# tohtsky/myFM

Hardware: AMD Instinct MI355X
Metric: Gibbs iterations/sec (rank=32) (higher is better)
Workload: dtype f64

## Files before the change

include/myfm_hip.h:

```cpp
#ifndef MYFM_HIP_H_
#define MYFM_HIP_H_

#include <stdint.h>

#ifdef __cplusplus
extern "C" {
#endif

#define MFM_OK 0
#define MFM_ERR_INVALID 1
#define MFM_ERR_RUNTIME 2
#define MFM_ERR_DEVICE 3

#define MFM_TASK_REGRESSION 0
#define MFM_TASK_CLASSIFICATION 1
#define MFM_TASK_ORDERED 2

typedef struct mfm_ctx mfm_ctx;
typedef struct mfm_design mfm_design;
typedef struct mfm_store mfm_store;

const char *mfm_version(void);
int mfm_device_count(void);
const char *mfm_global_error(void);
// ... 13 lines not shown
int mfm_comm_info(const mfm_ctx *ctx, int32_t *n_ranks, char *path, int64_t path_cap);
int mfm_peer_info(mfm_ctx *ctx, int32_t *pending, void **sum_buf, void **flag_buf, int64_t *sum_bytes, int64_t *flag_bytes);
int mfm_peer_set(mfm_ctx *ctx, int32_t world, int32_t rank, void *const *sum_bufs, void *const *flag_bufs);
int mfm_peer_model_info(mfm_ctx *ctx, void **w_buf, void **V_buf);
int mfm_peer_set_model(mfm_ctx *ctx, int32_t world, int32_t rank, void *const *w_bufs, void *const *V_bufs);
int mfm_peer_export(mfm_ctx *ctx, void *handles256);
int mfm_peer_import(mfm_ctx *ctx, int32_t world, int32_t rank, const void *all_handles);
int mfm_peer_drop(mfm_ctx *ctx);
int mfm_set_main_levels(mfm_ctx *ctx, const int32_t *level, int64_t D0);
int mfm_set_row_offset(mfm_ctx *ctx, int64_t first_global_row);

int mfm_set_main(mfm_ctx *ctx, int64_t N, int64_t D0, const int64_t *indptr, const int32_t *indices,
                 const double *data, const double *y);
int mfm_add_block(mfm_ctx *ctx, int64_t B, int64_t Db, const int64_t *indptr, const int32_t *indices,
                  const double *data, const int64_t *original_to_block);
int mfm_set_groups(mfm_ctx *ctx, const int32_t *group_index, int64_t D, int32_t G);
int mfm_set_residual_policy(mfm_ctx *ctx, int32_t recomputable);
int mfm_finalize(mfm_ctx *ctx, int32_t rank);

int64_t mfm_dim_all(const mfm_ctx *ctx);
int mfm_plan_info(const mfm_ctx *ctx, int64_t *n_levels_main, int64_t *n_launches_per_sweep);
int mfm_plan_flags(const mfm_ctx *ctx);
#define MFM_RES_INFO_FIELDS 16
int mfm_res_info(const mfm_ctx *ctx, int64_t *out, int n_out, char *why, int why_len);
#define MFM_CELL_INFO_FIELDS 74
int mfm_cell_info(const mfm_ctx *ctx, int64_t *out, int n_out, char *why, int why_len);
#define MFM_CHAIN_STREAM_INFO_FIELDS 30
int mfm_chain_stream_info(const mfm_ctx *ctx, int64_t *out, int max_records, int *n_records);

int mfm_set_state(mfm_ctx *ctx, double w0, const double *w, const double *V);
int mfm_get_state(mfm_ctx *ctx, double *w0, double *w, double *V);
int mfm_set_w0(mfm_ctx *ctx, double w0);
int mfm_zero_w(mfm_ctx *ctx);
int mfm_get_e(mfm_ctx *ctx, double *e);
int mfm_get_q(mfm_ctx *ctx, double *q);
int mfm_set_e(mfm_ctx *ctx, const double *e);

int mfm_reduce_e(mfm_ctx *ctx, double *sum_e, double *sum_e2);
int mfm_shift_e(mfm_ctx *ctx, double delta);
int mfm_group_stats_w(mfm_ctx *ctx, const double *mu_w, double *sum, double *ssd);
int mfm_group_stats_V(mfm_ctx *ctx, const double *mu_V, double *sum, double *ssd);
int mfm_hyper_stats(mfm_ctx *ctx, int32_t need_e, const double *mu_w, const double *mu_V, double *sum_e, double *sum_e2,
                    double *sum_w, double *ssd_w, double *sum_V, double *ssd_V);
int mfm_sweep_w(mfm_ctx *ctx, double alpha, const double *lambda_w, const double *mu_w, const double *z);
int mfm_sweep_V(mfm_ctx *ctx, int32_t f_begin, int32_t f_end, double alpha, const double *lambda_V,
                const double *mu_V, const double *z);
// ... 280 lines not shown
```

myfm_amd/_build.py:

```python
import os
import subprocess
import sys
import sysconfig

HERE = os.path.dirname(os.path.abspath(__file__))
ROOT = os.path.dirname(HERE)
CSRC = os.path.join(HERE, "csrc")
INCLUDE = os.path.join(ROOT, "include")
HIP_LIB = os.path.join(HERE, "libmyfm_hip.so")
EXT_SUFFIX = sysconfig.get_config_var("EXT_SUFFIX") or ".so"
PYMOD = os.path.join(HERE, "_myfm" + EXT_SUFFIX)

HIP_UNITS = {
    "mfm_hip.hip": ["mfm_env.hpp", "mfm_common.hpp", "mfm_wave.hpp", "mfm_policies.hpp", "mfm_kernels.hpp", "mfm_mf_kernels.hpp", "mfm_res.hpp", "mfm_res_entry.hpp", "mfm_res_plan.hpp",
                    "mfm_plan.hpp", "mfm_block_kernels.hpp", "mfm_erfcx.hpp", "mfm_tasks.hpp", "mfm_tn.hpp", "mfm_philox.hpp", "mfm_predict.hpp", "mfm_samples.hpp", "mfm_dist.hpp", "mfm_logdens.hpp", "mfm_psis.hpp", "mfm_ess.hpp", "mfm_crps.hpp", "mfm_loo_pred.hpp", "mfm_normal_quantile.hpp", "mfm_rng.hpp", "mfm_mtjump.hpp", "mfm_cell.hpp",
                    "mfm_chain_api.hpp", "mfm_rng_state.hpp", "mfm_latent_api.hpp", "mfm_latent_host.hpp", "mfm_comm.hpp", "mfm_vbmoments.hpp", "mfm_vb_sums.hpp"],
    "mfm_latent.hip": ["mfm_env.hpp", "mfm_common.hpp", "mfm_rng_state.hpp", "mfm_latent_api.hpp"],
    "mfm_cell.hip": ["mfm_env.hpp", "mfm_common.hpp", "mfm_wave.hpp", "mfm_cell.hpp"],
    "mfm_chain.hip": ["mfm_env.hpp", "mfm_common.hpp", "mfm_wave.hpp", "mfm_policies.hpp", "mfm_chain_api.hpp", "mfm_chain_plan.hpp", "mfm_chain_stream.hpp"],
    "mfm_vb.hip": ["mfm_env.hpp", "mfm_common.hpp", "mfm_erfcx.hpp", "mfm_vb.hpp", "mfm_comm.hpp"],
    "mfm_pairs.hip": ["mfm_env.hpp", "mfm_common.hpp", "mfm_pairs.hpp", "mfm_pairs_rank.hpp", "mfm_pairs_samples.hpp", "mfm_pairs_ucb.hpp", "mfm_pairs_vb.hpp", "mfm_vb_sums.hpp", "mfm_samples.hpp"],
    "mfm_foldin.hip": ["mfm_env.hpp", "mfm_common.hpp", "mfm_foldin.hpp", "mfm_foldin_handle.hpp", "mfm_philox.hpp", "mfm_samples.hpp"],
    "mfm_foldin_gibbs.hip": ["mfm_env.hpp", "mfm_common.hpp", "mfm_foldin.hpp", "mfm_foldin_gibbs.hpp", "mfm_foldin_gibbs_plan.hpp",
                             "mfm_foldin_handle.hpp", "mfm_tn.hpp", "mfm_philox.hpp", "mfm_samples.hpp"],
}
OBJ_DIR = os.path.join(CSRC, "_obj")
PYMOD_HEADERS = ["mfm_env.hpp", "mfm_hostnormals.hpp", "mfm_mtjump.hpp", "mfm_normal_quantile.hpp"]


def _newer(target, deps):
    if not os.path.exists(target):
        return True
    t = os.path.getmtime(target)
    return any(os.path.exists(d) and os.path.getmtime(d) > t for d in deps)


def _hipcc():
# ... 75 lines not shown
```

myfm_amd/_capi.py:

```python
import ctypes as C
import os

import numpy as np
import scipy.sparse as sps

_HERE = os.path.dirname(os.path.abspath(__file__))
LIB_PATH = os.path.join(_HERE, "libmyfm_hip.so")

MFM_OK, MFM_ERR_INVALID, MFM_ERR_RUNTIME, MFM_ERR_DEVICE = 0, 1, 2, 3
TASK_REGRESSION, TASK_CLASSIFICATION, TASK_ORDERED = 0, 1, 2

SYMBOLS = [
    "mfm_version", "mfm_device_count", "mfm_global_error", "mfm_create", "mfm_destroy", "mfm_last_error",
    "mfm_set_stream", "mfm_synchronize", "mfm_set_main", "mfm_add_block", "mfm_set_groups", "mfm_finalize",
    "mfm_peer_info", "mfm_peer_set", "mfm_peer_model_info", "mfm_peer_set_model", "mfm_peer_export", "mfm_peer_import", "mfm_peer_drop", "mfm_set_residual_policy", "mfm_dim_all", "mfm_plan_info", "mfm_plan_flags", "mfm_res_info", "mfm_cell_info", "mfm_chain_stream_info", "mfm_set_state", "mfm_get_state", "mfm_set_w0", "mfm_zero_w", "mfm_get_e",
    "mfm_get_q", "mfm_set_e", "mfm_reduce_e", "mfm_shift_e", "mfm_group_stats_w", "mfm_group_stats_V",
    "mfm_sweep_w", "mfm_sweep_V", "mfm_sweep_wV", "mfm_update_e_regression", "mfm_update_e_classification", "mfm_score_train",
    "mfm_oprobit_add_group", "mfm_oprobit_eval", "mfm_oprobit_sample_z", "mfm_hyper_stats", "mfm_timing_enable", "mfm_timing_select", "mfm_timing_reset",
    "mfm_timing_n_classes", "mfm_timing_class_name", "mfm_timing_get", "mfm_design_create", "mfm_design_add_block",
    "mfm_design_destroy", "mfm_design_last_error", "mfm_design_dim_all", "mfm_design_predict",
    "mfm_host_column_levels", "mfm_rng_prepare", "mfm_rng_seed_mt19937", "mfm_rng_set_program", "mfm_rng_prefetch", "mfm_rng_acquire",
    "mfm_rng_get_z", "mfm_design_score_ctx", "mfm_design_n_rows", "mfm_set_allreduce", "mfm_set_row_offset", "mfm_set_main_levels",
    "mfm_test_erfcx", "mfm_test_truncated_normal", "mfm_get_device", "mfm_set_shard", "mfm_comm_unique_id", "mfm_comm_init",
    "mfm_comm_stats", "mfm_comm_info", "mfm_store_create", "mfm_store_destroy", "mfm_store_last_error", "mfm_store_size", "mfm_store_push_ctx",
# ... 475 lines not shown
    def latent_stats(self):
        out = np.zeros(8, dtype=np.int64)
        self._ck(lib().mfm_latent_stats(self.h, _p(out)))
        return dict(zip(("status", "chunks", "subs", "lq", "quads", "walkers", "attempts"), (int(v) for v in out)))

    def rng_host_read(self, offset, n):
        out = np.empty(max(int(n), 1), dtype=np.uint32)
        self._ck(lib().mfm_rng_host_read(self.h, int(offset), int(n), _p(out)))
        return out[: int(n)]

    def rng_host_advance(self, words):
        self._ck(lib().mfm_rng_host_advance(self.h, int(words)))

    def set_residual_policy(self, recomputable):
        self._ck(lib().mfm_set_residual_policy(self.h, 1 if recomputable else 0))

    def plan_flags(self):
        f = lib().mfm_plan_flags(self.h)
        return {"qfree": bool(f & 1), "unit": bool(f & 2), "ell": bool(f & 4), "sharded": bool(f & 8), "soa": bool(f & 16),
                "fused_next": bool(f & 32), "sharded_fused": bool(f & 64), "mf": bool(f & 128), "resident": bool(f & 256), "cell": bool(f & 512), "streamed_chain": bool(f & 1024), "resident_overflow": bool(f & 2048)}

    RES_INFO = ("ready", "G", "RV", "RL", "RX", "umax", "n_items", "item_bits", "n_runs", "max_wg_users", "max_slice_items",
                "e_where", "n_rows", "s2_in_sweep_b", "lds_bytes", "entry_bytes")
    E_WHERE = ("rows", "slots", "slots_with_sums", "cell", "dropped")

    def res_info(self):
        out = np.zeros(len(self.RES_INFO), dtype=np.int64)
        why = C.create_string_buffer(256)
        self._ck(lib().mfm_res_info(self.h, _p(out), out.shape[0], why, len(why)))
        d = dict(zip(self.RES_INFO, (int(v) for v in out)))
        d["ready"] = bool(d["ready"])
        d["e_where"] = self.E_WHERE[d["e_where"]]
        d["why"] = why.value.decode()
        return d

    CELL_INFO = ("ready", "G", "umax", "item32", "n_streams", "n_fields", "N", "Npad", "max_steps", "chunk_max", "chunk_min",
                 "chunks_empty", "split_mask", "score_fb")
    CELL_STREAM_TYPE = ("U", "I", "C")
    CELL_MAX_STREAMS, CELL_MAX_FIELDS = 4, 16
    CELL_INFO_FIELDS = len(CELL_INFO) + 3 * CELL_MAX_STREAMS + 3 * CELL_MAX_FIELDS

    def cell_info(self):
        out = np.zeros(self.CELL_INFO_FIELDS, dtype=np.int64)
        why = C.create_string_buffer(256)
        self._ck(lib().mfm_cell_info(self.h, _p(out), out.shape[0], why, len(why)))
        n = len(self.CELL_INFO)
        nf = n + 3 * self.CELL_MAX_STREAMS
        d = dict(zip(self.CELL_INFO, (int(v) for v in out[:n])))
        d["ready"], d["item32"] = bool(d["ready"]), bool(d["item32"])
        d["streams"] = [(self.CELL_STREAM_TYPE[int(out[n + 3 * s])], int(out[n + 3 * s + 1]), int(out[n + 3 * s + 2]))
                        for s in range(d["n_streams"])]
        d["fields"] = [tuple(int(x) for x in out[nf + 3 * k:nf + 3 * k + 3]) for k in range(d["n_fields"])]
        d["why"] = why.value.decode()
# ... 614 lines not shown
```

myfm_amd/csrc/_myfm.cpp:

```cpp
#include <thread>
#include <cstdio>
#include <pybind11/functional.h>
#include <pybind11/numpy.h>
#include <pybind11/pybind11.h>
#include <pybind11/stl.h>

#include <algorithm>
#include <cmath>
#include <chrono>
#include <cstdint>
#include <cstdlib>
#include <functional>
#include <limits>
#include <memory>
#include <random>
#include <set>
#include <sstream>
#include <stdexcept>
#include <string>
#include <tuple>
#include <type_traits>
#include <vector>

#include "mfm_env.hpp"
// ... 3333 lines not shown
             mfm_comm_stats(s.trainer->ctx, &c, &d);
             return py::make_tuple(c, d);
           })
      .def("comm_info",
           [](GibbsSession &s) {
             int32_t n = 0;
             char path[512];
             if (mfm_comm_info(s.trainer->ctx, &n, path, sizeof(path)) != MFM_OK) throw std::runtime_error(mfm_global_error());
             return py::make_tuple((int)n, std::string(path));
           },
           "(ranks of the library's own RCCL communicator (ncclCommCount), path of the librccl.so it bound); (0, '') without one")
      .def("step", &GibbsSession::step, py::call_guard<py::gil_scoped_release>())
      .def("synchronize", &GibbsSession::synchronize)
      .def("residual", &GibbsSession::residual)
      .def("timing_enable", &GibbsSession::timing_enable)
      .def("timing_select", &GibbsSession::timing_select)
      .def("timing_reset", &GibbsSession::timing_reset)
      .def("timing", &GibbsSession::timing)
      .def("plan_info", &GibbsSession::plan_info)
      .def("latent_info", &GibbsSession::latent_info)
      .def("plan_flags", [](GibbsSession &s) { return mfm_plan_flags(s.trainer->ctx); })
      .def("res_info",
           [](GibbsSession &s) {
             std::vector<int64_t> v(MFM_RES_INFO_FIELDS, 0);
             ck(s.trainer->ctx, mfm_res_info(s.trainer->ctx, v.data(), (int)v.size(), nullptr, 0));
             return v;
           },
           "the persistent sweep's layout: the MFM_RES_INFO_FIELDS values of mfm_res_info (myfm_hip.h)")
      .def("peer_info",
           [](GibbsSession &s) {
             int32_t pending = 0;
             void *sum = nullptr, *flag = nullptr;
             int64_t sb = 0, fb = 0;
             ck(s.trainer->ctx, mfm_peer_info(s.trainer->ctx, &pending, &sum, &flag, &sb, &fb));
             return py::make_tuple(pending != 0, (uintptr_t)sum, (uintptr_t)flag, sb, fb);
           })
      .def("peer_set",
           [](GibbsSession &s, int world, int rank, const std::vector<uintptr_t> &sums, const std::vector<uintptr_t> &flags) {
             if ((int)sums.size() != world || (int)flags.size() != world) throw std::invalid_argument("peer_set: one buffer pair per rank");
             std::vector<void *> a, b;
             for (auto v : sums) a.push_back((void *)v);
             for (auto v : flags) b.push_back((void *)v);
             ck(s.trainer->ctx, mfm_peer_set(s.trainer->ctx, world, rank, a.data(), b.data()));
           })
      .def("peer_model_info",
           [](GibbsSession &s) {
             void *w = nullptr, *V = nullptr;
             ck(s.trainer->ctx, mfm_peer_model_info(s.trainer->ctx, &w, &V));
             return py::make_tuple((uintptr_t)w, (uintptr_t)V);
           })
      .def("peer_set_model",
// ... 135 lines not shown
```

myfm_amd/csrc/mfm_hip.hip:

```cpp
#include <algorithm>
#include <cerrno>
#include <chrono>
#include <cmath>
#include <cstdio>
#include <cstring>
#include <map>
#include <memory>
#include <mutex>
#include <string>
#include <thread>
#include <type_traits>
#include <vector>

#include <fcntl.h>
#include <sys/file.h>
#include <sys/stat.h>
#include <unistd.h>

#include <hipcub/hipcub.hpp>

#include "mfm_common.hpp"
#include "mfm_kernels.hpp"
#include "mfm_plan.hpp"
#include "mfm_res_plan.hpp"
// ... 1528 lines not shown
  bool streamed = false;
  for (auto &B : ctx->blocks)
    for (const Step &st : B->plan_V.steps) streamed = streamed || (st.is_chain && st.chain.form == ChainForm::Stream);
  int form = 0;
  switch (ctx->v_path) {
    case VPath::QFree: form = 1; break;
    case VPath::Split: form = 16; break;
    case VPath::SplitFused: form = 16 | 32; break;
    case VPath::TwoField: form = 16 | 32 | 128; break;
    case VPath::ShardedSplit: form = 64; break;
    case VPath::ShardedTwoField: form = 64 | 128; break;
    case VPath::Deferred:
    case VPath::Generic:
    case VPath::Cell:
      break;
  }
  return (streamed ? 1024 : 0) | (ctx->resident_V() && ctx->res.RX > 0 ? 2048 : 0) | form | (ctx->X.unit ? 2 : 0) | (ctx->X.ell_width >= 0 ? 4 : 0) |
         (ctx->comm.active() ? 8 : 0) | (ctx->resident_V() ? 256 : 0) | (ctx->cell.ready ? 512 : 0);
}

int mfm_res_info(const mfm_ctx *ctx, int64_t *out, int n_out, char *why, int why_len) {
  if (!ctx || n_out < 0 || (n_out > 0 && !out) || why_len < 0 || (why_len > 0 && !why)) return MFM_ERR_INVALID;
  const ResPlan &rp = ctx->res;
  const int64_t v[MFM_RES_INFO_FIELDS] = {ctx->resident_V() ? 1 : 0, rp.G,       rp.RV,     rp.RL,           rp.RX,
                                          rp.umax,          rp.n_items, rp.item_bits, rp.n_runs,    rp.max_wg_users,
                                          rp.max_slice_items, (int64_t)ctx->e_where, rp.n_rows, rp.s2b, (int64_t)rp.lds_bytes,
                                          rp.ent_bytes};
  for (int i = 0; i < n_out; i++) out[i] = i < MFM_RES_INFO_FIELDS ? v[i] : 0;
  if (why_len > 0) {
    std::strncpy(why, ctx->resident_V() ? "" : rp.why.c_str(), (size_t)why_len - 1);
    why[why_len - 1] = 0;
  }
  return MFM_OK;
}

int mfm_cell_info(const mfm_ctx *ctx, int64_t *out, int n_out, char *why, int why_len) {
  if (!ctx || n_out < 0 || (n_out > 0 && !out) || why_len < 0 || (why_len > 0 && !why)) return MFM_ERR_INVALID;
  const CellPlan &cp = ctx->cell;
  int64_t v[MFM_CELL_INFO_FIELDS] = {0};
  const int m = (int)cp.fields.size(), ns = (int)cp.streams.size();
  int64_t split = 0;
  const bool typed = ns > 0 && cp.sU == 0;
  for (int k = 0; k < m && typed; k++)
    if (cp.split_pass(k == 0 ? m - 1 : k - 1, k, k == 0)) split |= (int64_t)1 << k;
  const int64_t head[14] = {cp.ready ? 1 : 0, cp.G,         cp.umax,      cp.item32 ? 1 : 0, ns,    m, cp.N, cp.Npad, cp.max_steps,
                            cp.chunk_max,     cp.chunk_min, cp.chunks_empty, split,          cp.ready ? cp.score_fb() : 0};
  for (int i = 0; i < 14; i++) v[i] = head[i];
  for (int i = 0; i < ns && i < CELL_MAX_STREAMS; i++) {
    v[14 + 3 * i] = cp.streams[i].type;
    v[15 + 3 * i] = cp.streams[i].slot;
    v[16 + 3 * i] = cp.streams[i].card;
// ... 938 lines not shown
```

myfm_amd/csrc/mfm_res.hpp:

```cpp
#pragma once
#include <algorithm>
#include <cstdlib>
#include <cstring>
#include <atomic>
#include <string>
#include <thread>
#include <type_traits>
#include <vector>

#include "mfm_common.hpp"
#include "mfm_mf_kernels.hpp"
#include "mfm_res_entry.hpp"

namespace mfm {

#ifndef MFM_RES_CH
#define MFM_RES_CH 4
#endif
constexpr int RES_MAX_PEERS = 8;

struct ResArgs {
  double2 *eq;
  const double *e_in;
  double *e_slots;
  const int32_t *perm;
  const uint32_t *uidw;
  const uint32_t *headw;
  const int32_t *run_item;
  const int32_t *first_run;
  const int32_t *wg_run_ptr;
  const int32_t *wg_nruns;
  const int32_t *wg_user_ptr;
  const int2 *user_desc;
  const int32_t *wg_item_ptr;
// ... 1045 lines not shown
  void alloc_exchange(int world, int rank, hipStream_t s) {
    xworld = world;
    xrank = rank;
    peers_set = false;
    peers_model = false;
    xepoch = 0;
    auto alloc_shared = [&](auto &buf, size_t count) {
      buf.release();
      void *p = nullptr;
      const size_t bytes = count * sizeof(*buf.p);
      if (hipExtMallocWithFlags(&p, bytes, hipDeviceMallocUncached) != hipSuccess) {
        (void)hipGetLastError();
        throw Error(MFM_ERR_DEVICE, "no uncached device memory for the ranks' exchange buffers (hipExtMallocWithFlags(hipDeviceMallocUncached))");
      }
      buf.p = (decltype(buf.p))p;
      buf.n = count;
      buf.owned = true;
      MFM_HIP_CHECK(hipMemsetAsync(p, 0, bytes, s));
    };
    alloc_shared(xsum, xsum_bytes(world) / sizeof(double));
    alloc_shared(xflag, (size_t)16 * RES_MAX_PEERS);
    xarrive.alloc_zero(16, s);
  }
  std::string why;
  std::vector<int32_t> h_nruns;
  std::vector<std::string> h_diag;

  static int bits_for(int64_t n) {
    int b = 1;
    while (((int64_t)1 << b) < n) b++;
    return b;
  }
  struct Variant {
    int rv, rl;
  };
  static std::vector<Variant> variants() {
    std::vector<Variant> v;
    for (const ResForm &f : res_forms())
      if (!f.xch && !f.ovf && !f.s2b) v.push_back({f.rv, f.rl});
    return v;
  }

  bool choose_layout(int64_t N, const std::vector<int64_t> &ustart, int64_t max_user, int n_cu, std::vector<int64_t> &ucut) {
    const int64_t n_users = (int64_t)ustart.size() - 1;
    const std::vector<Variant> vs = variants();
    const int nv = (int)vs.size();
// ... 213 lines not shown
      for (int32_t c : wg_run_item[g]) h_slot_ptr[(size_t)c + 1]++;
    }
    for (int c = 0; c < n_items; c++) h_slot_ptr[(size_t)c + 1] += h_slot_ptr[c];
    h_slot_ptr[n_items] = (int32_t)counter;
    n_runs = counter;
    if (counter >= ((int64_t)1 << 31) - 2) return fail("too many runs");
    std::vector<int32_t> run_base = run_bases(nruns);
    const int32_t zero_run = run_base[G];
    std::vector<int32_t> h_run_item((size_t)zero_run + 1, n_items);
    for (int g = 0; g < G; g++) {
      std::copy(wg_run_item[g].begin(), wg_run_item[g].end(), h_run_item.begin() + run_base[g]);
      if (fill[g] < cap_slots) {
        const int th = (int)(fill[g] / R), rh = (int)(fill[g] % R);
        h_headw[((size_t)g * HW + rh / 16) * NT + th] |= 1u << (rh % 16);
      }
      h_headw[((size_t)g * HW) * NT] |= 1u;
      for (int t = 0; t < NT; t++) {
        const int64_t s0 = (int64_t)t * R;
        int32_t &fr = h_first[(size_t)g * NT + t];
        fr = (s0 >= fill[g] ? nruns[g] : fr) + run_base[g];
      }
    }
    std::vector<int32_t> h_uptr((size_t)G + 1, 0);
    std::vector<int2> h_udesc;
    for (int g = 0; g < G; g++) {
      for (int32_t j : wg_users[g]) h_udesc.push_back(make_int2(j, group_of && (size_t)j < group_of->size() ? (*group_of)[j] : 0));
      h_uptr[g + 1] = (int32_t)h_udesc.size();
    }
    std::vector<int32_t> h_iptr;
    if (!choose_item_slices(h_slot_ptr, counter, h_iptr)) return false;
    int imax = 0;
    for (int g = 0; g < G; g++) imax = std::max(imax, h_iptr[g + 1] - h_iptr[g]);
    max_slice_items = imax;
    umax = std::max(maxu, imax) + 1;
    if (umax > 1024) return fail("internal: user field");
    std::vector<uint32_t> h_uidw((size_t)G * UW * NT, 0);
    res_parallel_for(G, [&](int g) {
      for (int64_t sl = 0; sl < cap_slots; sl++) {
        const uint16_t u16 = h_uid[(size_t)g * cap_slots + (size_t)sl];
        const uint32_t u = u16 == 0xffffu ? (uint32_t)(umax - 1) : u16;
        const int t = (int)(sl / R), r = (int)(sl % R);
        const int w0 = 5 * (r / 16), bb = (r % 16) / 4, k = r % 4;
        if (k < 3) {
          h_uidw[((size_t)g * UW + w0 + bb) * NT + t] |= u << (10 * k);
        } else {
          h_uidw[((size_t)g * UW + w0 + bb) * NT + t] |= (u & 3u) << 30;
          h_uidw[((size_t)g * UW + w0 + 4) * NT + t] |= (u >> 2) << (8 * bb);
        }
      }
    });
    h_uid = std::vector<uint16_t>();
    std::vector<int32_t> slice_of((size_t)n_items);
    for (int g = 0; g < G; g++)
      for (int c = h_iptr[g]; c < h_iptr[g + 1]; c++) slice_of[c] = g;
    std::vector<int32_t> h_eptr((size_t)G + 1, 0);
    {
      std::vector<int64_t> cnt((size_t)G, 0);
      for (int g = 0; g < G; g++)
        for (int32_t c : wg_run_item[g]) cnt[slice_of[c]]++;
      for (int g = 0; g < G; g++) {
        const int64_t e = h_eptr[g] + ((cnt[g] + WAVE - 1) / WAVE) * WAVE;
        if (e >= ((int64_t)1 << 31)) return fail("too many entries");
        h_eptr[g + 1] = (int32_t)e;
// ... 376 lines not shown
```

myfm_amd/csrc/mfm_res_plan.hpp:

```cpp
#pragma once
#include <chrono>

#include <hipcub/hipcub.hpp>

#include "mfm_res.hpp"

namespace mfm {

namespace rp {

constexpr int TB = 256;

__global__ void k_rows(const int32_t *__restrict__ colidx, int64_t N, int32_t *__restrict__ bflag, int32_t *__restrict__ ucnt,
                       int32_t *__restrict__ icnt, int32_t *__restrict__ red) {
  const int64_t r = (int64_t)blockIdx.x * blockDim.x + threadIdx.x;
  int32_t mu = -1, mi = 0x7fffffff;
  if (r < N) {
    const int2 c = ((const int2 *)colidx)[r];
    const bool b = r == 0 || c.x != colidx[2 * (r - 1)];
    bflag[r] = b ? 1 : 0;
    if (b) atomicAdd(&ucnt[c.x], 1);
    atomicAdd(&icnt[c.y], 1);
    mu = c.x;
    mi = c.y;
// ... 111 lines not shown
                       const int32_t *__restrict__ hrun0, const int32_t *__restrict__ run_base, int item_bits, int64_t N,
                       int32_t *__restrict__ run_item_c, int32_t *__restrict__ run_item, int32_t *__restrict__ runs_per_item) {
  const int64_t p = (int64_t)blockIdx.x * blockDim.x + threadIdx.x;
  if (p >= N || !headf[p]) return;
  const uint32_t k = key[p];
  const int g = (int)(k >> item_bits);
  const int32_t item = (int32_t)(k & ((1u << item_bits) - 1u));
  const int32_t kc = hs[p] - 1;
  run_item_c[kc] = item;
  run_item[run_base[g] + kc - hrun0[g]] = item;
  atomicAdd(&runs_per_item[item], 1);
}

__global__ void k_first(const int32_t *__restrict__ hs, const int32_t *__restrict__ rowcut, const int32_t *__restrict__ hrun0,
                        const int32_t *__restrict__ run_base, int G, int R, int NT, int32_t *__restrict__ first_run) {
  const int i = blockIdx.x * blockDim.x + threadIdx.x;
  if (i >= G * NT) return;
  const int g = i / NT, t = i % NT;
  const int32_t fill = rowcut[g + 1] - rowcut[g], s0 = t * R;
  const int32_t nr = hrun0[g + 1] - hrun0[g];
  first_run[i] = run_base[g] + (s0 >= fill ? nr : hs[rowcut[g] + s0] - 1 - hrun0[g]);
}

__global__ void k_pack(const uint16_t *__restrict__ uid, const int32_t *__restrict__ headf, const int32_t *__restrict__ rowcut, int G, int R,
                       int NT, int umax, uint32_t *__restrict__ uidw, uint32_t *__restrict__ headw) {
  const int HW = R / 16, UW = 5 * HW;
  const int64_t i = (int64_t)blockIdx.x * blockDim.x + threadIdx.x;
  if (i >= (int64_t)G * HW * NT) return;
  const int t = (int)(i % NT), grp = (int)((i / NT) % HW), g = (int)(i / ((int64_t)NT * HW));
  const int64_t cap = (int64_t)R * NT;
  const int32_t fill = rowcut[g + 1] - rowcut[g];
  uint32_t w[5] = {0, 0, 0, 0, 0}, hw = 0;
  for (int q = 0; q < 16; q++) {
    const int32_t sidx = t * R + 16 * grp + q;
    const uint16_t u16 = uid[(int64_t)g * cap + sidx];
    const uint32_t u = u16 == 0xffffu ? (uint32_t)(umax - 1) : u16;
    const int bb = q / 4, k = q % 4;
    if (k < 3) {
      w[bb] |= u << (10 * k);
    } else {
      w[bb] |= (u & 3u) << 30;
      w[4] |= (u >> 2) << (8 * bb);
    }
    const bool head = sidx < fill ? headf[rowcut[g] + sidx] != 0 : sidx == fill;
    if (head || sidx == 0) hw |= 1u << q;
  }
  for (int k = 0; k < 5; k++) uidw[((int64_t)g * UW + 5 * grp + k) * NT + t] = w[k];
  headw[((int64_t)g * HW + grp) * NT + t] = hw;
}

__global__ void k_user_desc(const int32_t *__restrict__ users, const int32_t *__restrict__ empties, const int32_t *__restrict__ ucut,
                            const int32_t *__restrict__ uptr, const int32_t *__restrict__ group, int G, int32_t n_users, int32_t n_emp,
                            int2 *__restrict__ desc) {
  __shared__ int32_t cut[1026];
  for (int i = threadIdx.x; i <= G; i += blockDim.x) cut[i] = ucut[i];
  __syncthreads();
  const int32_t i = blockIdx.x * blockDim.x + threadIdx.x;
  if (i < n_users) {
    const int g = upper_group(cut, G, i);
    const int32_t j = users[i];
    desc[uptr[g] + (i - cut[g])] = make_int2(j, group ? group[j] : 0);
  } else if (i < n_users + n_emp) {
    const int32_t k = i - n_users;
    const int g = k % G;
    const int32_t j = empties[k];
    desc[uptr[g] + (cut[g + 1] - cut[g]) + k / G] = make_int2(j, group ? group[j] : 0);
  }
}

__global__ void k_item_desc(const int32_t *__restrict__ scols, const int32_t *__restrict__ group, int32_t n_items, int2 *__restrict__ desc) {
  const int32_t i = blockIdx.x * blockDim.x + threadIdx.x;
  if (i < n_items) desc[i] = make_int2(scols[i], group ? group[scols[i]] : 0);
}

__global__ void k_run_feat(const int32_t *__restrict__ run_item, const int32_t *__restrict__ scols, int32_t n_items, int64_t n_run_item,
                           int64_t n, int32_t *__restrict__ run_feat) {
  const int64_t r = (int64_t)blockIdx.x * blockDim.x + threadIdx.x;
  if (r >= n) return;
  int32_t f = -1;
  if (r < n_run_item) {
    const int32_t c = run_item[r];
    if (c < n_items) f = scols[c];
  }
  run_feat[r] = f;
}

__global__ void k_slice_keys(const int32_t *__restrict__ run_item_c, const int32_t *__restrict__ iptr, int G, int64_t n, uint32_t *__restrict__ key,
                             int32_t *__restrict__ val) {
  __shared__ int32_t cut[1026];
// ... 193 lines not shown
  rpn.wg_run_ptr.upload(run_base);
  rpn.wg_nruns.upload(nruns);
  rpn.run_item.alloc((size_t)zero_run + 1);
  hipLaunchKernelGGL(k_fill32, grid(zero_run + 1), dim3(TB), 0, s, rpn.run_item.p, (int64_t)zero_run + 1, n_items);
  DevBuf<int32_t> run_item_c, runs_per_item;
  run_item_c.alloc((size_t)std::max<int64_t>(counter, 1));
  runs_per_item.alloc_zero((size_t)n_items, s);
  hipLaunchKernelGGL(k_runs, grid(N), dim3(TB), 0, s, key2.p, headf.p, hs.p, hrun0.p, rpn.wg_run_ptr.p, rpn.item_bits, N, run_item_c.p,
                     rpn.run_item.p, runs_per_item.p);
  rpn.first_run.alloc((size_t)G * NT);
  hipLaunchKernelGGL(k_first, grid((int64_t)G * NT), dim3(TB), 0, s, hs.p, rowcut.p, hrun0.p, rpn.wg_run_ptr.p, G, R, NT, rpn.first_run.p);
  lap("slots, heads, runs, first");
  std::vector<int32_t> h_slot_ptr((size_t)n_items + 1, 0), h_iptr;
  {
    const std::vector<int32_t> rpi = download(runs_per_item.p, (size_t)n_items, s);
    for (int c = 0; c < n_items; c++) h_slot_ptr[(size_t)c + 1] = h_slot_ptr[c] + rpi[c];
  }
  if (!rpn.choose_item_slices(h_slot_ptr, counter, h_iptr)) return false;
  int imax = 0;
  for (int g = 0; g < G; g++) imax = std::max(imax, h_iptr[g + 1] - h_iptr[g]);
  rpn.max_slice_items = imax;
  rpn.umax = std::max(maxu, imax) + 1;
  if (rpn.umax > 1024) return rpn.fail("internal: user field");
  const int UW = 5 * (R / 16), HW = R / 16;
  rpn.uidw.alloc((size_t)G * UW * NT);
  rpn.headw.alloc((size_t)G * HW * NT);
  hipLaunchKernelGGL(k_pack, grid((int64_t)G * HW * NT), dim3(TB), 0, s, uid.p, headf.p, rowcut.p, G, R, NT, rpn.umax, rpn.uidw.p, rpn.headw.p);
  std::vector<int32_t> h_eptr((size_t)G + 1, 0), h_sstart((size_t)G + 1, 0);
  for (int g = 0; g < G; g++) {
    const int64_t cnt = h_slot_ptr[h_iptr[g + 1]] - h_slot_ptr[h_iptr[g]];
    const int64_t e = h_eptr[g] + ((cnt + WAVE - 1) / WAVE) * WAVE;
    if (e >= ((int64_t)1 << 31)) return rpn.fail("too many entries");
    h_eptr[g + 1] = (int32_t)e;
    h_sstart[g + 1] = h_sstart[g] + (int32_t)cnt;
  }
  rpn.wg_item_ptr.upload(h_iptr);
  rpn.ent_ptr.upload(h_eptr);
  rpn.choose_entry_width(zero_run);
  const bool ent4 = rpn.ent_bytes == 4;
  rpn.entries.alloc((size_t)(rpn.ent_bytes / 4) * (size_t)h_eptr[G]);
  if (h_eptr[G]) hipLaunchKernelGGL(k_fill_entries, grid(h_eptr[G]), dim3(TB), 0, s, rpn.entries.p, (int64_t)h_eptr[G], zero_run, 0, ent4);
  if (counter > 0) {
    DevBuf<int32_t> sstart;
    sstart.upload(h_sstart);
    DevBuf<uint32_t> sk, sk2;
    DevBuf<int32_t> sv, sv2;
    sk.alloc((size_t)counter);
    sk2.alloc((size_t)counter);
    sv.alloc((size_t)counter);
    sv2.alloc((size_t)counter);
    hipLaunchKernelGGL(k_slice_keys, grid(counter), dim3(TB), 0, s, run_item_c.p, rpn.wg_item_ptr.p, G, counter, sk.p, sv.p);
    sort_pairs(sk, sk2, sv, sv2, counter, gbits, tmp, s);
    hipLaunchKernelGGL(k_entries, grid(counter), dim3(TB), 0, s, sk2.p, sv2.p, run_item_c.p, hrun0.p, rpn.wg_run_ptr.p, rpn.wg_item_ptr.p,
                       rpn.ent_ptr.p, sstart.p, G, counter, rpn.entries.p, ent4);
    MFM_HIP_CHECK(hipStreamSynchronize(s));
  }
  lap("slices, pack, entries");
  DevBuf<int32_t> d_group;
  if (group_of && (int64_t)group_of->size() >= D0) d_group.upload(group_of->data(), (size_t)D0);
  rpn.user_desc.alloc((size_t)h_uptr[G]);
  hipLaunchKernelGGL(k_user_desc, grid((int64_t)n_users + n_emp), dim3(TB), 0, s, d_users.p, empties.p, d_ucut.p, rpn.wg_user_ptr.p, d_group.p, G,
                     n_users, n_emp, rpn.user_desc.p);
  rpn.item_desc.alloc((size_t)n_items);
  hipLaunchKernelGGL(k_item_desc, grid(n_items), dim3(TB), 0, s, rpn.scols.p, d_group.p, n_items, rpn.item_desc.p);
  rpn.run_feat.alloc((size_t)zero_run + 1 + 8);
  hipLaunchKernelGGL(k_run_feat, grid((int64_t)zero_run + 9), dim3(TB), 0, s, rpn.run_item.p, rpn.scols.p, n_items, (int64_t)zero_run + 1,
                     (int64_t)zero_run + 9, rpn.run_feat.p);
  {
    std::vector<int32_t> h_fill((size_t)G);
    for (int g = 0; g < G; g++) h_fill[g] = h_rowcut[g + 1] - h_rowcut[g];
    rpn.wg_fill.upload(h_fill);
  }
  if (!rpn.plan_lds()) return rpn.fail("LDS");
  rpn.fill_s2_lin(s);
  rpn.e_slots.alloc((size_t)G * cap_slots);
  rpn.sums.alloc((size_t)G);
  rpn.y_slots = DevBuf<double>();
  rpn.h_nruns = nruns;
  rpn.h_diag.clear();
  rpn.partials.alloc((size_t)2 * ((size_t)zero_run + 1));
  MFM_HIP_CHECK(hipMemsetAsync(rpn.partials.p, 0, (size_t)16 * ((size_t)zero_run + 1), s));
  rpn.dv.alloc((size_t)rpn.dv_doubles() * (n_items + 1));
  rpn.bar.alloc(RES_BAR_WORDS);
  MFM_HIP_CHECK(hipStreamSynchronize(s));
  MFM_HIP_CHECK(hipGetLastError());
  lap("descriptors, buffers");
  rpn.ready = true;
  rpn.why.clear();
  return true;
}

static inline std::string res_plan_compare(const ResPlan &a, const ResPlan &b, hipStream_t s) {
  if (a.G != b.G || a.RV != b.RV || a.RL != b.RL || a.RX != b.RX || a.umax != b.umax || a.item_bits != b.item_bits || a.n_items != b.n_items ||
      a.n_rows != b.n_rows || a.n_runs != b.n_runs || a.lds_bytes != b.lds_bytes || a.s2b != b.s2b || a.max_wg_users != b.max_wg_users ||
      a.max_slice_items != b.max_slice_items || a.ent_bytes != b.ent_bytes)
    return "scalars";
  auto same = [&](const void *p, size_t np, const void *q, size_t nq, size_t elem) {
    if (np != nq) return false;
    std::vector<char> x(np * elem), y(nq * elem);
    if (np) {
      MFM_HIP_CHECK(hipMemcpyAsync(x.data(), p, np * elem, hipMemcpyDeviceToHost, s));
      MFM_HIP_CHECK(hipMemcpyAsync(y.data(), q, nq * elem, hipMemcpyDeviceToHost, s));
    }
    MFM_HIP_CHECK(hipStreamSynchronize(s));
    return x == y;
  };
#define MFM_RP_CMP(f) \
  if (!same(a.f.p, a.f.n, b.f.p, b.f.n, sizeof(*a.f.p))) return #f;
  MFM_RP_CMP(perm)
  MFM_RP_CMP(first_run)
  MFM_RP_CMP(wg_run_ptr)
  MFM_RP_CMP(wg_nruns)
  MFM_RP_CMP(wg_user_ptr)
  MFM_RP_CMP(wg_item_ptr)
  MFM_RP_CMP(ent_ptr)
  MFM_RP_CMP(scols)
  MFM_RP_CMP(entries)
  MFM_RP_CMP(uidw)
// ... 13 lines not shown
```

Baseline: 380.6.

## Renumber per-workgroup user slots to reduce LDS bank conflicts in resident sweep

Adds a host-side greedy assignment that renumbers each workgroup's users so their LDS positions spread across banks. It uses a model of the gfx950 LDS access groups for 64-bit reads, 128-bit reads and 64-bit atomic adds. The packed uid words and user descriptors are rewritten through this numbering, so the persistent sweep kernel's LDS accumulations conflict less. This adds planning time on the host and a device-to-host download of uid, and exposes conflict counts in res_info. An env flag can keep the identity numbering.

Result: faster. 385.1 (median of 5 runs) (+1.2%).

```diff
diff --git a/include/myfm_hip.h b/include/myfm_hip.h
--- a/include/myfm_hip.h
+++ b/include/myfm_hip.h
@@ -59,6 +59,7 @@
 int mfm_plan_info(const mfm_ctx *ctx, int64_t *n_levels_main, int64_t *n_launches_per_sweep);
 int mfm_plan_flags(const mfm_ctx *ctx);
 #define MFM_RES_INFO_FIELDS 16
+#define MFM_RES_INFO_BANK_FIELDS 2
 int mfm_res_info(const mfm_ctx *ctx, int64_t *out, int n_out, char *why, int why_len);
 #define MFM_CELL_INFO_FIELDS 74
 int mfm_cell_info(const mfm_ctx *ctx, int64_t *out, int n_out, char *why, int why_len);
diff --git a/myfm_amd/_build.py b/myfm_amd/_build.py
--- a/myfm_amd/_build.py
+++ b/myfm_amd/_build.py
@@ -12,7 +12,7 @@
 PYMOD = os.path.join(HERE, "_myfm" + EXT_SUFFIX)
 
 HIP_UNITS = {
-    "mfm_hip.hip": ["mfm_env.hpp", "mfm_common.hpp", "mfm_wave.hpp", "mfm_policies.hpp", "mfm_kernels.hpp", "mfm_mf_kernels.hpp", "mfm_res.hpp", "mfm_res_entry.hpp", "mfm_res_plan.hpp",
+    "mfm_hip.hip": ["mfm_env.hpp", "mfm_common.hpp", "mfm_wave.hpp", "mfm_policies.hpp", "mfm_kernels.hpp", "mfm_mf_kernels.hpp", "mfm_res.hpp", "mfm_res_banks.hpp", "mfm_res_entry.hpp", "mfm_res_plan.hpp",
                     "mfm_plan.hpp", "mfm_block_kernels.hpp", "mfm_erfcx.hpp", "mfm_tasks.hpp", "mfm_tn.hpp", "mfm_philox.hpp", "mfm_predict.hpp", "mfm_samples.hpp", "mfm_dist.hpp", "mfm_logdens.hpp", "mfm_psis.hpp", "mfm_ess.hpp", "mfm_crps.hpp", "mfm_loo_pred.hpp", "mfm_normal_quantile.hpp", "mfm_rng.hpp", "mfm_mtjump.hpp", "mfm_cell.hpp",
                     "mfm_chain_api.hpp", "mfm_rng_state.hpp", "mfm_latent_api.hpp", "mfm_latent_host.hpp", "mfm_comm.hpp", "mfm_vbmoments.hpp", "mfm_vb_sums.hpp"],
     "mfm_latent.hip": ["mfm_env.hpp", "mfm_common.hpp", "mfm_rng_state.hpp", "mfm_latent_api.hpp"],
diff --git a/myfm_amd/_capi.py b/myfm_amd/_capi.py
--- a/myfm_amd/_capi.py
+++ b/myfm_amd/_capi.py
@@ -521,13 +521,14 @@
 
     RES_INFO = ("ready", "G", "RV", "RL", "RX", "umax", "n_items", "item_bits", "n_runs", "max_wg_users", "max_slice_items",
                 "e_where", "n_rows", "s2_in_sweep_b", "lds_bytes", "entry_bytes")
+    RES_INFO_BANKS = ("bank_cycles_identity", "bank_cycles_chosen")
     E_WHERE = ("rows", "slots", "slots_with_sums", "cell", "dropped")
 
     def res_info(self):
-        out = np.zeros(len(self.RES_INFO), dtype=np.int64)
+        out = np.zeros(len(self.RES_INFO) + len(self.RES_INFO_BANKS), dtype=np.int64)
         why = C.create_string_buffer(256)
         self._ck(lib().mfm_res_info(self.h, _p(out), out.shape[0], why, len(why)))
-        d = dict(zip(self.RES_INFO, (int(v) for v in out)))
+        d = dict(zip(self.RES_INFO + self.RES_INFO_BANKS, (int(v) for v in out)))
         d["ready"] = bool(d["ready"])
         d["e_where"] = self.E_WHERE[d["e_where"]]
         d["why"] = why.value.decode()
diff --git a/myfm_amd/csrc/_myfm.cpp b/myfm_amd/csrc/_myfm.cpp
--- a/myfm_amd/csrc/_myfm.cpp
+++ b/myfm_amd/csrc/_myfm.cpp
@@ -3379,11 +3379,11 @@
       .def("plan_flags", [](GibbsSession &s) { return mfm_plan_flags(s.trainer->ctx); })
       .def("res_info",
            [](GibbsSession &s) {
-             std::vector<int64_t> v(MFM_RES_INFO_FIELDS, 0);
+             std::vector<int64_t> v(MFM_RES_INFO_FIELDS + MFM_RES_INFO_BANK_FIELDS, 0);
              ck(s.trainer->ctx, mfm_res_info(s.trainer->ctx, v.data(), (int)v.size(), nullptr, 0));
              return v;
            },
-           "the persistent sweep's layout: the MFM_RES_INFO_FIELDS values of mfm_res_info (myfm_hip.h)")
+           "the persistent sweep's layout: the MFM_RES_INFO_FIELDS + MFM_RES_INFO_BANK_FIELDS values of mfm_res_info (myfm_hip.h)")
       .def("peer_info",
            [](GibbsSession &s) {
              int32_t pending = 0;
diff --git a/myfm_amd/csrc/mfm_hip.hip b/myfm_amd/csrc/mfm_hip.hip
--- a/myfm_amd/csrc/mfm_hip.hip
+++ b/myfm_amd/csrc/mfm_hip.hip
@@ -1574,11 +1574,12 @@
 int mfm_res_info(const mfm_ctx *ctx, int64_t *out, int n_out, char *why, int why_len) {
   if (!ctx || n_out < 0 || (n_out > 0 && !out) || why_len < 0 || (why_len > 0 && !why)) return MFM_ERR_INVALID;
   const ResPlan &rp = ctx->res;
-  const int64_t v[MFM_RES_INFO_FIELDS] = {ctx->resident_V() ? 1 : 0, rp.G,       rp.RV,     rp.RL,           rp.RX,
-                                          rp.umax,          rp.n_items, rp.item_bits, rp.n_runs,    rp.max_wg_users,
-                                          rp.max_slice_items, (int64_t)ctx->e_where, rp.n_rows, rp.s2b, (int64_t)rp.lds_bytes,
-                                          rp.ent_bytes};
-  for (int i = 0; i < n_out; i++) out[i] = i < MFM_RES_INFO_FIELDS ? v[i] : 0;
+  constexpr int NF = MFM_RES_INFO_FIELDS + MFM_RES_INFO_BANK_FIELDS;
+  const int64_t v[NF] = {ctx->resident_V() ? 1 : 0, rp.G,       rp.RV,     rp.RL,           rp.RX,
+                         rp.umax,          rp.n_items, rp.item_bits, rp.n_runs,    rp.max_wg_users,
+                         rp.max_slice_items, (int64_t)ctx->e_where, rp.n_rows, rp.s2b, (int64_t)rp.lds_bytes,
+                         rp.ent_bytes,     rp.bank_add_identity, rp.bank_add_chosen};
+  for (int i = 0; i < n_out; i++) out[i] = i < NF ? v[i] : 0;
   if (why_len > 0) {
     std::strncpy(why, ctx->resident_V() ? "" : rp.why.c_str(), (size_t)why_len - 1);
     why[why_len - 1] = 0;
diff --git a/myfm_amd/csrc/mfm_res.hpp b/myfm_amd/csrc/mfm_res.hpp
--- a/myfm_amd/csrc/mfm_res.hpp
+++ b/myfm_amd/csrc/mfm_res.hpp
@@ -10,6 +10,7 @@
 
 #include "mfm_common.hpp"
 #include "mfm_mf_kernels.hpp"
+#include "mfm_res_banks.hpp"
 #include "mfm_res_entry.hpp"
 
 namespace mfm {
@@ -1101,6 +1102,29 @@
     alloc_shared(xflag, (size_t)16 * RES_MAX_PEERS);
     xarrive.alloc_zero(16, s);
   }
+  int64_t bank_add_identity = 0, bank_add_chosen = 0;
+  void number_users(const std::vector<uint16_t> &h_uid, const std::vector<int32_t> &h_uptr, std::vector<uint16_t> &num) {
+    const int Rt = R();
+    const size_t cap_slots = (size_t)NT * Rt;
+    const bool identity = env_flag("MFM_RES_BANKS_IDENTITY");
+    num.assign((size_t)G * NT, 0);
+    std::vector<int64_t> c_id((size_t)G, 0), c_ch((size_t)G, 0);
+    res_parallel_for(G, [&](int g) {
+      const int nu = h_uptr[g + 1] - h_uptr[g];
+      const uint16_t *uid_g = h_uid.data() + (size_t)g * cap_slots;
+      uint16_t *num_g = num.data() + (size_t)g * NT;
+      for (int u = 0; u < nu; u++) num_g[u] = (uint16_t)u;
+      c_id[g] = c_ch[g] = res_bank_count(uid_g, NT, Rt, nullptr, umax - 1).a_add;
+      if (identity) return;
+      res_bank_number(uid_g, NT, Rt, nu, umax - 1, num_g);
+      c_ch[g] = res_bank_count(uid_g, NT, Rt, num_g, umax - 1).a_add;
+    });
+    bank_add_identity = bank_add_chosen = 0;
+    for (int g = 0; g < G; g++) {
+      bank_add_identity += c_id[g];
+      bank_add_chosen += c_ch[g];
+    }
+  }
   std::string why;
   std::vector<int32_t> h_nruns;
   std::vector<std::string> h_diag;
@@ -1360,11 +1384,7 @@
       }
     }
     std::vector<int32_t> h_uptr((size_t)G + 1, 0);
-    std::vector<int2> h_udesc;
-    for (int g = 0; g < G; g++) {
-      for (int32_t j : wg_users[g]) h_udesc.push_back(make_int2(j, group_of && (size_t)j < group_of->size() ? (*group_of)[j] : 0));
-      h_uptr[g + 1] = (int32_t)h_udesc.size();
-    }
+    for (int g = 0; g < G; g++) h_uptr[g + 1] = h_uptr[g] + (int32_t)wg_users[g].size();
     std::vector<int32_t> h_iptr;
     if (!choose_item_slices(h_slot_ptr, counter, h_iptr)) return false;
     int imax = 0;
@@ -1372,11 +1392,19 @@
     max_slice_items = imax;
     umax = std::max(maxu, imax) + 1;
     if (umax > 1024) return fail("internal: user field");
+    std::vector<uint16_t> num;
+    number_users(h_uid, h_uptr, num);
+    std::vector<int2> h_udesc((size_t)h_uptr[G]);
+    for (int g = 0; g < G; g++)
+      for (size_t k = 0; k < wg_users[g].size(); k++) {
+        const int32_t j = wg_users[g][k];
+        h_udesc[(size_t)h_uptr[g] + num[(size_t)g * NT + k]] = make_int2(j, group_of && (size_t)j < group_of->size() ? (*group_of)[j] : 0);
+      }
     std::vector<uint32_t> h_uidw((size_t)G * UW * NT, 0);
     res_parallel_for(G, [&](int g) {
       for (int64_t sl = 0; sl < cap_slots; sl++) {
         const uint16_t u16 = h_uid[(size_t)g * cap_slots + (size_t)sl];
-        const uint32_t u = u16 == 0xffffu ? (uint32_t)(umax - 1) : u16;
+        const uint32_t u = u16 == RES_UID_PAD ? (uint32_t)(umax - 1) : num[(size_t)g * NT + u16];
         const int t = (int)(sl / R), r = (int)(sl % R);
         const int w0 = 5 * (r / 16), bb = (r % 16) / 4, k = r % 4;
         if (k < 3) {
diff --git a/myfm_amd/csrc/mfm_res_banks.hpp b/myfm_amd/csrc/mfm_res_banks.hpp
--- /dev/null
+++ b/myfm_amd/csrc/mfm_res_banks.hpp
@@ -0,0 +1,151 @@
+#pragma once
+#include <algorithm>
+#include <cstdint>
+#include <vector>
+
+namespace mfm {
+
+constexpr int RES_BANK_POS = 16;
+constexpr uint16_t RES_UID_PAD = 0xffffu;
+
+enum ResLdsOp { RES_LDS_READ64 = 0, RES_LDS_READ128 = 1, RES_LDS_ADD64 = 2 };
+
+inline int res_lds_groups(ResLdsOp op) { return op == RES_LDS_READ64 ? 2 : 4; }
+inline int res_lds_group(ResLdsOp op, int l) {
+  if (op == RES_LDS_READ64) return l >> 5;
+  if (op == RES_LDS_ADD64) return l >> 4;
+  const int m = l & 31;
+  const int odd = (m >= 4 && m < 12) || (m >= 16 && m < 20) || m >= 28 ? 1 : 0;
+  return 2 * (l >> 5) + odd;
+}
+
+inline int res_lds_extra_cycles(ResLdsOp op, const uint32_t addr[64]) {
+  const int nbanks = op == RES_LDS_ADD64 ? 32 : 64, dwords = op == RES_LDS_READ128 ? 4 : 2, ng = res_lds_groups(op);
+  int extra = 0;
+  for (int grp = 0; grp < ng; grp++) {
+    int worst = 0;
+    for (int b = 0; b < nbanks; b++) {
+      uint32_t seen[64];
+      int n = 0;
+      for (int l = 0; l < 64; l++) {
+        if (res_lds_group(op, l) != grp) continue;
+        bool touches = false;
+        for (int d = 0; d < dwords; d++) touches = touches || (int)((addr[l] / 4 + d) % nbanks) == b;
+        if (!touches) continue;
+        bool dup = false;
+        if (op != RES_LDS_ADD64)
+          for (int i = 0; i < n; i++) dup = dup || seen[i] == addr[l];
+        if (!dup) seen[n++] = addr[l];
+      }
+      worst = std::max(worst, n);
+    }
+    extra += worst > 0 ? worst - 1 : 0;
+  }
+  return extra;
+}
+
+struct ResBankCycles {
+  int64_t a_add = 0;
+  int64_t a_read = 0;
+  int64_t b_read = 0;
+  int64_t b_add = 0;
+  int64_t b() const { return b_read + b_add; }
+};
+
+inline ResBankCycles res_bank_count(const uint16_t *uid, int NT, int R, const uint16_t *num, int pad) {
+  ResBankCycles c;
+  for (int w = 0; w < NT / 64; w++)
+    for (int r = 0; r < R; r++) {
+      int idx[64];
+      for (int l = 0; l < 64; l++) {
+        const uint16_t u = uid[(size_t)(64 * w + l) * R + r];
+        idx[l] = u == RES_UID_PAD ? pad : num ? (int)num[u] : (int)u;
+      }
+      for (int op = 0; op < 3; op++) {
+        const int ng = res_lds_groups((ResLdsOp)op);
+        for (int grp = 0; grp < ng; grp++) {
+          int seen[RES_BANK_POS][32], n[RES_BANK_POS] = {0};
+          int worst = 0;
+          for (int l = 0; l < 64; l++) {
+            if (res_lds_group((ResLdsOp)op, l) != grp) continue;
+            const int p = idx[l] % RES_BANK_POS;
+            bool dup = false;
+            if (op != RES_LDS_ADD64)
+              for (int i = 0; i < n[p]; i++) dup = dup || seen[p][i] == idx[l];
+            if (!dup) seen[p][n[p]++] = idx[l];
+            worst = std::max(worst, n[p]);
+          }
+          const int extra = worst > 0 ? worst - 1 : 0;
+          if (op == RES_LDS_READ64) c.a_read += extra;
+          if (op == RES_LDS_READ128) c.b_read += extra;
+          if (op == RES_LDS_ADD64) c.a_add += extra;
+        }
+      }
+    }
+  c.b_add = c.a_add;
+  return c;
+}
+
+inline void res_bank_number(const uint16_t *uid, int NT, int R, int nu, int pad, uint16_t *num) {
+  const int NW = NT / 64, P = RES_BANK_POS;
+  const size_t nq = (size_t)NW * R * 4, nh = (size_t)NW * R * 2;
+  std::vector<int32_t> ptr((size_t)nu + 1, 0);
+  for (size_t s = 0; s < (size_t)NT * R; s++)
+    if (uid[s] != RES_UID_PAD) ptr[(size_t)uid[s] + 1]++;
+  for (int u = 0; u < nu; u++) ptr[(size_t)u + 1] += ptr[u];
+  std::vector<int32_t> at(ptr.begin(), ptr.end() - 1), qs((size_t)ptr[nu]);
+  std::vector<uint8_t> cq(nq * P, 0), mq(nq, 0);
+  std::vector<uint8_t> ch(nh * P, 0), mh(nh, 0);
+  const int pp = pad % P;
+  for (int w = 0; w < NW; w++)
+    for (int r = 0; r < R; r++)
+      for (int l = 0; l < 64; l++) {
+        const uint16_t u = uid[(size_t)(64 * w + l) * R + r];
+        const size_t q = ((size_t)w * R + r) * 4 + (l >> 4);
+        if (u != RES_UID_PAD) {
+          qs[(size_t)at[u]++] = (int32_t)q;
+        } else {
+          mq[q] = std::max(mq[q], ++cq[q * P + pp]);
+          ch[(q >> 1) * P + pp] = 1;
+          mh[q >> 1] = std::max<uint8_t>(mh[q >> 1], 1);
+        }
+      }
+  std::vector<int32_t> order((size_t)nu);
+  for (int u = 0; u < nu; u++) order[u] = u;
+  std::stable_sort(order.begin(), order.end(), [&](int32_t x, int32_t y) { return ptr[x + 1] - ptr[x] > ptr[y + 1] - ptr[y]; });
+  int used[RES_BANK_POS] = {0}, room[RES_BANK_POS];
+  for (int p = 0; p < P; p++) room[p] = nu > p ? (nu - p + P - 1) / P : 0;
+  for (int32_t u : order) {
+    const int32_t *b = qs.data() + ptr[u], *e = qs.data() + ptr[u + 1];
+    int best = -1;
+    int64_t best_add = 0, best_read = 0;
+    for (int p = 0; p < P; p++) {
+      if (used[p] >= room[p]) continue;
+      int64_t d_add = 0, d_read = 0;
+      int32_t h_prev = -1;
+      for (const int32_t *i = b; i < e;) {
+        const int32_t q = *i;
+        int m = 0;
+        for (; i < e && *i == q; i++) m++;
+        d_add += std::max(0, (int)cq[(size_t)q * P + p] + m - (int)mq[q]);
+        if ((q >> 1) != h_prev)
+          d_read += std::max(0, (int)ch[(size_t)(q >> 1) * P + p] + 1 - (int)mh[q >> 1]);
+        h_prev = q >> 1;
+      }
+      if (best < 0 || d_add < best_add || (d_add == best_add && d_read < best_read)) {
+        best = p;
+        best_add = d_add;
+        best_read = d_read;
+      }
+    }
+    const int p = best;
+    num[u] = (uint16_t)(p + P * used[p]++);
+    for (const int32_t *i = b; i < e; i++) {
+      const int32_t q = *i;
+      mq[q] = std::max(mq[q], ++cq[(size_t)q * P + p]);
+      if (i == b || (*(i - 1) >> 1) != (q >> 1)) mh[q >> 1] = std::max(mh[q >> 1], ++ch[(size_t)(q >> 1) * P + p]);
+    }
+  }
+}
+
+}
diff --git a/myfm_amd/csrc/mfm_res_plan.hpp b/myfm_amd/csrc/mfm_res_plan.hpp
--- a/myfm_amd/csrc/mfm_res_plan.hpp
+++ b/myfm_amd/csrc/mfm_res_plan.hpp
@@ -157,8 +157,9 @@
   first_run[i] = run_base[g] + (s0 >= fill ? nr : hs[rowcut[g] + s0] - 1 - hrun0[g]);
 }
 
-__global__ void k_pack(const uint16_t *__restrict__ uid, const int32_t *__restrict__ headf, const int32_t *__restrict__ rowcut, int G, int R,
-                       int NT, int umax, uint32_t *__restrict__ uidw, uint32_t *__restrict__ headw) {
+__global__ void k_pack(const uint16_t *__restrict__ uid, const uint16_t *__restrict__ num, const int32_t *__restrict__ headf,
+                       const int32_t *__restrict__ rowcut, int G, int R, int NT, int umax, uint32_t *__restrict__ uidw,
+                       uint32_t *__restrict__ headw) {
   const int HW = R / 16, UW = 5 * HW;
   const int64_t i = (int64_t)blockIdx.x * blockDim.x + threadIdx.x;
   if (i >= (int64_t)G * HW * NT) return;
@@ -169,7 +170,7 @@
   for (int q = 0; q < 16; q++) {
     const int32_t sidx = t * R + 16 * grp + q;
     const uint16_t u16 = uid[(int64_t)g * cap + sidx];
-    const uint32_t u = u16 == 0xffffu ? (uint32_t)(umax - 1) : u16;
+    const uint32_t u = u16 == RES_UID_PAD ? (uint32_t)(umax - 1) : num[(int64_t)g * NT + u16];
     const int bb = q / 4, k = q % 4;
     if (k < 3) {
       w[bb] |= u << (10 * k);
@@ -185,8 +186,8 @@
 }
 
 __global__ void k_user_desc(const int32_t *__restrict__ users, const int32_t *__restrict__ empties, const int32_t *__restrict__ ucut,
-                            const int32_t *__restrict__ uptr, const int32_t *__restrict__ group, int G, int32_t n_users, int32_t n_emp,
-                            int2 *__restrict__ desc) {
+                            const int32_t *__restrict__ uptr, const uint16_t *__restrict__ num, const int32_t *__restrict__ group, int G,
+                            int NT, int32_t n_users, int32_t n_emp, int2 *__restrict__ desc) {
   __shared__ int32_t cut[1026];
   for (int i = threadIdx.x; i <= G; i += blockDim.x) cut[i] = ucut[i];
   __syncthreads();
@@ -194,12 +195,12 @@
   if (i < n_users) {
     const int g = upper_group(cut, G, i);
     const int32_t j = users[i];
-    desc[uptr[g] + (i - cut[g])] = make_int2(j, group ? group[j] : 0);
+    desc[uptr[g] + num[(int64_t)g * NT + (i - cut[g])]] = make_int2(j, group ? group[j] : 0);
   } else if (i < n_users + n_emp) {
     const int32_t k = i - n_users;
     const int g = k % G;
     const int32_t j = empties[k];
-    desc[uptr[g] + (cut[g + 1] - cut[g]) + k / G] = make_int2(j, group ? group[j] : 0);
+    desc[uptr[g] + num[(int64_t)g * NT + (cut[g + 1] - cut[g]) + k / G]] = make_int2(j, group ? group[j] : 0);
   }
 }
 
@@ -439,10 +440,18 @@
   rpn.max_slice_items = imax;
   rpn.umax = std::max(maxu, imax) + 1;
   if (rpn.umax > 1024) return rpn.fail("internal: user field");
+  DevBuf<uint16_t> d_num;
+  {
+    std::vector<uint16_t> h_num;
+    rpn.number_users(download(uid.p, (size_t)G * cap_slots, s), h_uptr, h_num);
+    d_num.upload(h_num);
+  }
+  lap("user numbering");
   const int UW = 5 * (R / 16), HW = R / 16;
   rpn.uidw.alloc((size_t)G * UW * NT);
   rpn.headw.alloc((size_t)G * HW * NT);
-  hipLaunchKernelGGL(k_pack, grid((int64_t)G * HW * NT), dim3(TB), 0, s, uid.p, headf.p, rowcut.p, G, R, NT, rpn.umax, rpn.uidw.p, rpn.headw.p);
+  hipLaunchKernelGGL(k_pack, grid((int64_t)G * HW * NT), dim3(TB), 0, s, uid.p, d_num.p, headf.p, rowcut.p, G, R, NT, rpn.umax, rpn.uidw.p,
+                     rpn.headw.p);
   std::vector<int32_t> h_eptr((size_t)G + 1, 0), h_sstart((size_t)G + 1, 0);
   for (int g = 0; g < G; g++) {
     const int64_t cnt = h_slot_ptr[h_iptr[g + 1]] - h_slot_ptr[h_iptr[g]];
@@ -476,8 +485,8 @@
   DevBuf<int32_t> d_group;
   if (group_of && (int64_t)group_of->size() >= D0) d_group.upload(group_of->data(), (size_t)D0);
   rpn.user_desc.alloc((size_t)h_uptr[G]);
-  hipLaunchKernelGGL(k_user_desc, grid((int64_t)n_users + n_emp), dim3(TB), 0, s, d_users.p, empties.p, d_ucut.p, rpn.wg_user_ptr.p, d_group.p, G,
-                     n_users, n_emp, rpn.user_desc.p);
+  hipLaunchKernelGGL(k_user_desc, grid((int64_t)n_users + n_emp), dim3(TB), 0, s, d_users.p, empties.p, d_ucut.p, rpn.wg_user_ptr.p, d_num.p,
+                     d_group.p, G, NT, n_users, n_emp, rpn.user_desc.p);
   rpn.item_desc.alloc((size_t)n_items);
   hipLaunchKernelGGL(k_item_desc, grid(n_items), dim3(TB), 0, s, rpn.scols.p, d_group.p, n_items, rpn.item_desc.p);
   rpn.run_feat.alloc((size_t)zero_run + 1 + 8);
@@ -510,7 +519,8 @@
 static inline std::string res_plan_compare(const ResPlan &a, const ResPlan &b, hipStream_t s) {
   if (a.G != b.G || a.RV != b.RV || a.RL != b.RL || a.RX != b.RX || a.umax != b.umax || a.item_bits != b.item_bits || a.n_items != b.n_items ||
       a.n_rows != b.n_rows || a.n_runs != b.n_runs || a.lds_bytes != b.lds_bytes || a.s2b != b.s2b || a.max_wg_users != b.max_wg_users ||
-      a.max_slice_items != b.max_slice_items || a.ent_bytes != b.ent_bytes)
+      a.max_slice_items != b.max_slice_items || a.ent_bytes != b.ent_bytes || a.bank_add_identity != b.bank_add_identity ||
+      a.bank_add_chosen != b.bank_add_chosen)
     return "scalars";
   auto same = [&](const void *p, size_t np, const void *q, size_t nq, size_t elem) {
     if (np != nq) return false;
```
